# RaulAstudillo06/BOCF

Hardware: AMD Instinct MI355X
Metric: acquisition evals/sec (candidates x MC-samples/sec), uEI_noiseless batch call; GP-fit ms alongside (higher is better)
Workload: dtype f64; 1 GPU; BASELINE configs[2]: m=4 rbf-ARD GP, N=4096 d=8, S=1024 MC samples, C=65536 candidates, noise 1e-06, top-16 selection; N=4096, d=8, m=4, S=1024, C=65536, rccl_ranks_seen=0

## Files before the change

### bocf_amd/csrc/bocf_ctx.h

```cpp
#pragma once
#include "bocf_internal.h"
#include "chol_plan.h"
#include "predict_plan.h"
#include "../../include/bocf_hip.h"

#include <map>
#include <string>
#include <utility>
#include <vector>

void bocf_set_error(const char* text);
int bocf_launch_status();
int bocf_plan_cholesky(bocf_ctx* c, bool kinv, CholPlan* out);
int bocf_run_cholesky(bocf_ctx* c, const CholPlan& plan, bool counters_zeroed = false);
int bocf_run_trtri(bocf_ctx* c, bool early_done);
int bocf_comm_broadcast(bocf_ctx* c, double* buf, size_t count, int root);
int bocf_comm_group(bool start);
int bocf_comm_abort(bocf_ctx* c);
int bocf_comm_allreduce_sum(bocf_ctx* c, double* buf, size_t count);
#define fail bocf_fail
#define HIPCHK(expr)                                                         \
  do {                                                                       \
    hipError_t e_ = (expr);                                                  \
    if (e_ != hipSuccess) return fail(#expr, hipGetErrorString(e_));         \
// ... 8 lines not shown
static inline int nsplit_for(int Np, int Cpad, int m) {
  const int blocks = ((Cpad + 511) / 512) * m;
  int ns = 2048 / (blocks > 0 ? blocks : 1);
  if (ns < 1) ns = 1;
  const int maxs = Np / BOCF_TILE;
  if (ns > maxs) ns = maxs;
  return ns;
}



static_assert(PLAN_TILE == BOCF_TILE && PLAN_SMALL_N == BOCF_SMALL_N && PLAN_I8_SLICES == BOCF_I8_SLICES, "predict_plan.h mirrors bocf_internal.h");

struct DevBuf {
  void* p = nullptr;
  size_t cap = 0;
  int ensure(size_t bytes) {
    if (bytes <= cap) return 0;
    if (p) (void)hipFree(p);
    p = nullptr;
    cap = 0;
    hipError_t e = hipMalloc(&p, bytes);
    if (e != hipSuccess) return fail("hipMalloc", hipGetErrorString(e));
    cap = bytes;
    return 0;
  }
  void release() {
    if (p) (void)hipFree(p);
    p = nullptr;
    cap = 0;
  }
  template <typename T> T* as() const { return reinterpret_cast<T*>(p); }
};

struct bocf_ctx {
  int device = 0;
  hipStream_t stream = nullptr;
  void* pin_in = nullptr; void* pin_out = nullptr;
  size_t pin_in_cap = 0, pin_out_cap = 0;
  hipEvent_t ev_pin = nullptr;
  void* fit_pin = nullptr; size_t fit_pin_cap = 0;
  void* up_pin = nullptr; size_t up_pin_cap = 0, arena_used = 0;
  std::vector<hipEvent_t> ev_chol;
  hipStream_t s_res = nullptr, s_hi = nullptr, s_bulk = nullptr;
  DevBuf chol_flags;
  int chol_flags_used = 0;
  int chol_err_off = 0;
  CholOptions chol;
  int kinv_done = 0;
  int inverse_done = 0;
  int ncu = 0;
  int* tile_ctr = nullptr;
  unsigned long long* team_tl = nullptr;
  int res_cus = 0;
  int cu_masks_ok = 1;
  hipStream_t s_inv = nullptr;
  hipEvent_t ev_half = nullptr, ev_inv_early = nullptr;
  int early_inverse_started = 0;
  void* zeroed_R = nullptr; void* zeroed_RT = nullptr; int zeroed_Np = 0, zeroed_m = 0;
  int gated_off = 0;
  long long sched_timeouts = 0;
  int sched_retry = 0;
  long long fits_done = 0;
  int last_schedule = 0;
  int sched_m = 0;
  int force_sched_timeout = 0;
  int data_N = 0, data_d = 0, data_m = 0;
  int fused_infer = 1;
  int reuse_data = 0;
  int skip_mu_train = 0;
  DevBuf gpart, gout;
  DevBuf hmc_buf;
  double* infer_out = nullptr;
  size_t infer_out_cap = 0;
  bool fitted = false;
  bool canned = false;
  int N = 0, Np = 0, d = 0, m = 0, kernel_id = 0;
  long xs_stride = 0;
  std::vector<int> kernel_ids;
  std::vector<int> pending_ids;
  std::vector<KernHyp> hyp;
  std::vector<double> jitter;
  std::vector<int> last_info;
  DevBuf R32;
  bool r32_valid = false;
  int predict_f32 = 0;
  DevBuf Ri8, Ri8e, Ki8, Ki8e;
  bool ri8_valid = false;
  int predict_i8 = 0, i8_group = 0;
  DevBuf X, Xs, S, R, RT, E, ET, T, yc, tvec, rvec, dvec, alpha, lml, jit, hypd, info, mu_train;
  int C = 0;
  DevBuf Xc;
  long chunk = 65536;
  long workspace_mb = 24576;
  DevBuf Kstar, meanpart, sumsq, mean, var, acq, Vbuf, dmean, dvar, dacq, Vs, Ws;
  int pred_cap = 0;
  DevBuf theta, prob, best, params, Wt;
  std::vector<double> last_params;
  long long mu_epoch = 0;
  long long best_epoch = -1; int best_sig = -1;
  int S_mc = 0;
  bool have_acq = false;
  DevBuf prog_buf;
  UtilProg prog;
  DevBuf blk_idx, blk_val, out_idx, out_val;
  DevBuf eu_theta, eu_rows, eu_Z, eu_val, eu_grad;
// ... 120 lines not shown
```

### bocf_amd/csrc/bocf_internal.h

```cpp
#pragma once
#include <hip/hip_runtime.h>
#include <stdint.h>
#include "kern_dispatch.h"
#include "util_args.h"

#define BOCF_TILE 128
#define BOCF_MAX_FITS 1024

void bocf_note_launch(const char* kernel, hipError_t e);
#define BOCF_LAUNCH(kern, grid, block, shm, stream, ...)              \
  do {                                                                \
    hipLaunchKernelGGL(kern, grid, block, shm, stream, __VA_ARGS__);  \
    bocf_note_launch(#kern, hipGetLastError());                       \
  } while (0)
template <typename F>
static inline void bocf_launch_by_d(const char* kernel, int d, F f) {
  if (!bocf_dispatch_d(d, f)) bocf_note_launch(kernel, hipErrorInvalidValue);
}

__device__ __forceinline__ void dd_fma_acc(double& s, double& c, double a, double b) {
#pragma clang fp contract(off)
  const double p = a * b;
  const double e = __builtin_fma(a, b, -p);
  const double t = s + p;
// ... 1 lines not shown
  c += ((s - (t - z)) + (p - z)) + e;
  s = t;
}
__device__ __forceinline__ void dd_add_acc(double& s, double& c, double hi, double lo) {
#pragma clang fp contract(off)
  const double t = s + hi;
  const double z = t - s;
  c += ((s - (t - z)) + (hi - z)) + lo;
  s = t;
}

__device__ __forceinline__ double bocf_exp_nonpos_times(double x, double a) {
  x = __builtin_fmax(x, -1100.0);
  const double dn = __builtin_rint(x * 0x1.71547652b82fep+0);
  const double t = __builtin_fma(-dn, 0x1.abc9e3b39803fp-56, __builtin_fma(-dn, 0x1.62e42fefa39efp-1, x));
  double p = __builtin_fma(t, 0x1.ade156a5dcb37p-26, 0x1.28af3fca7ab0cp-22);
  p = __builtin_fma(t, p, 0x1.71dee623fde64p-19);
  p = __builtin_fma(t, p, 0x1.a01997c89e6b0p-16);
  p = __builtin_fma(t, p, 0x1.a01a014761f6ep-13);
  p = __builtin_fma(t, p, 0x1.6c16c1852b7b0p-10);
  p = __builtin_fma(t, p, 0x1.1111111122322p-7);
  p = __builtin_fma(t, p, 0x1.55555555502a1p-5);
  p = __builtin_fma(t, p, 0x1.5555555555511p-3);
  p = __builtin_fma(t, p, 0x1.000000000000bp-1);
  p = __builtin_fma(t, p, 1.0);
  p = __builtin_fma(t, p, 1.0);
  return __builtin_ldexp(a * p, (int)dn);
}
__device__ __forceinline__ double bocf_exp_nonpos(double x) { return bocf_exp_nonpos_times(x, 1.0); }

struct GemmArgs {
  const double* A;  long lda;  long strideA;
  const double* B;  long ldb;  long strideB;
  const double* Cin; double* Cout; long ldc; long strideC;
  int M, Ncols, K;
  int kb, krt, kct;
  int kbeg_rt, kbeg_ct;
  int batch1;
  long strideA2, strideB2, strideC2;
  int upper_only;
  int rt_desc;
  int ct_desc;
  int swizzle;
  int batch;
  int prefetch1;
  int stagger;
  int no_x3;
  int vprobe;
  double alpha, beta;
  double* sumsq;
  long strideSumsq;
  int* tile_ctr;
  int ncu;
};
void launch_gemm_f64(const GemmArgs& g, int batch, int epilogue, hipStream_t s);

struct GemmArgs32 {
  const float* A; long lda; long strideA;
  const float* B; long ldb; long strideB;
  int M, Ncols, K;
  double* sumsq; long strideSumsq;
  int tile128;
};
void launch_gemm_f32_sumsq(const GemmArgs32& g, int batch, hipStream_t s);
void launch_f64_to_f32(const double* src, float* dst, long n, hipStream_t s);

struct KernHyp {
  double variance;
  double noise;
  double ymean;
  double ls[BOCF_MAX_D];
  double jitter;
};

void launch_scale_inputs(const double* X, int n, int d, const KernHyp* hyp, int m, double* Xs, long strideXs, hipStream_t s);
void launch_build_train_kernel(const double* Xs, long strideXs, int N, int Np, int d, int kernel_id, const KernHyp* hyp,
                               const double* jitter, int add_diag, double* S, long strideS, int m, hipStream_t s, const int* kids = nullptr);
void launch_tile128(const double* A, long lda, long strideA, const double* B, long ldb, long strideB, double* C, long ldc, long strideC,
                    double alpha, double beta, int m, hipStream_t s, int ntiles = 1, int K = 128, int* done = nullptr);
#ifdef BOCF_PROBES
void dbg_tl_start();
void dbg_tl_dump(const char* path);
#endif
void set_potrf_scalar(int on);
void launch_potrf_diag(double* S, long strideS, int N, int Np, int p, double* E, double* ET, long strideE, int* info, int m, hipStream_t s,
                       int* done = nullptr);
void launch_gate(const int* f0, int n0, const int* f1, int n1, int* err, hipStream_t s);
void launch_signal(int* f, int add, hipStream_t s);
struct TeamArgs {
  double* S; double* RT; double* R; long strideS;
  double* E; double* ET; long strideE;
  int N, Np, nb;
  int* info;
  int* F; int fstride;
  int* err;
  int T;
  int p0, p1;
  int do_inverse;
  double* KI; int do_kinv;
  int crit_load;
  int stream;
  unsigned long long* tl;
};
void launch_chol_team(const TeamArgs& a, int m, hipStream_t s);
#define BOCF_INFER_MAX_D 16
void launch_infer128(const double* X, int N, int d, int kernel_id, const KernHyp* hyp, const double* yc, double* out, int m, hipStream_t s,
// ... 323 lines not shown
```

### bocf_amd/csrc/capi.hip

```cpp
#include "bocf_ctx.h"

#include <chrono>
#include <cmath>
#include <cstdio>
#include <cstdlib>
#include <cstring>
#include <string>
#include <vector>

static thread_local std::string g_err;
int bocf_fail(const char* what, const char* detail) {
  g_err = std::string(what) + ": " + (detail ? detail : "");
  return -1;
}
void bocf_set_error(const char* text) { g_err = text ? text : ""; }

static thread_local std::string g_launch_err;
void bocf_note_launch(const char* kernel, hipError_t e) {
  if (e != hipSuccess && g_launch_err.empty()) g_launch_err = std::string("launch of ") + kernel + ": " + hipGetErrorString(e);
}
int bocf_launch_status() {
  const hipError_t e = hipGetLastError();
  if (!g_launch_err.empty()) {
    g_err = g_launch_err;
// ... 38 lines not shown
  *out = c;
  return 0;
}

static void drop_events(bocf_ctx* c) {
  for (auto& pr : c->events) {
    (void)hipEventDestroy(pr.first);
    (void)hipEventDestroy(pr.second);
  }
  c->events.clear();
}

static void drop_phases(bocf_ctx* c) {
  for (auto& kv : c->phases)
    for (auto& pr : kv.second) {
      (void)hipEventDestroy(pr.first);
      (void)hipEventDestroy(pr.second);
    }
  c->phases.clear();
}

extern "C" void bocf_destroy(bocf_ctx* c) {
  if (!c) return;
  (void)hipSetDevice(c->device);
  (void)hipStreamSynchronize(c->stream);
  (void)bocf_comm_destroy(c);
  if (c->shard_helper) bocf_destroy(c->shard_helper);
  c->shard_helper = nullptr;
  if (c->ts_helper) bocf_destroy(c->ts_helper);
  c->ts_helper = nullptr;
  for (DevBuf& b : c->ts_F) b.release();
  for (DevBuf& b : c->pt_buf) b.release();
  drop_events(c);
  drop_phases(c);
  if (c->pin_in) (void)hipHostFree(c->pin_in);
  if (c->pin_out) (void)hipHostFree(c->pin_out);
  if (c->fit_pin) (void)hipHostFree(c->fit_pin);
  if (c->up_pin) (void)hipHostFree(c->up_pin);
  if (c->ev_pin) (void)hipEventDestroy(c->ev_pin);
  if (c->eu_pin) (void)hipHostFree(c->eu_pin);
  if (c->ev_eu_pin) (void)hipEventDestroy(c->ev_eu_pin);
  DevBuf* bufs[] = {&c->R32, &c->Ri8, &c->Ri8e, &c->Ki8, &c->Ki8e, &c->X, &c->Xs, &c->S, &c->R, &c->RT, &c->E, &c->ET, &c->T, &c->yc, &c->tvec, &c->alpha, &c->lml, &c->jit, &c->hypd,
                    &c->info, &c->mu_train, &c->rvec, &c->dvec, &c->hmc_buf, &c->Xc, &c->Kstar, &c->meanpart, &c->sumsq, &c->mean, &c->var, &c->acq, &c->Vbuf, &c->dmean, &c->dvar, &c->dacq, &c->Vs, &c->Ws, &c->theta,
                    &c->prob, &c->best, &c->params, &c->Wt, &c->blk_idx, &c->blk_val, &c->out_idx, &c->out_val, &c->gpart, &c->gout, &c->pack, &c->gidx,
                    &c->gval, &c->shard_meta, &c->chol_flags, &c->eu_theta, &c->eu_rows, &c->eu_Z, &c->eu_val, &c->eu_grad,
                    &c->ts_X, &c->ts_K, &c->ts_V, &c->ts_mp, &c->ts_mu, &c->ts_Z, &c->ts_jit, &c->ts_u, &c->ts_theta, &c->ts_params, &c->ts_out,
                    &c->kg_XA, &c->kg_VA, &c->kg_Wa, &c->kg_muA, &c->kg_s2A, &c->kg_nug, &c->kg_V, &c->kg_W, &c->kg_cov, &c->kg_s2c, &c->kg_dcov, &c->kg_dmean, &c->kg_dvar,
                    &c->kg_par, &c->kg_v0, &c->kg_astar, &c->kg_AB, &c->kg_out, &c->kg_dout, &c->prog_buf,
                    &c->pd_XP, &c->pd_VP, &c->pd_Wp, &c->pd_muP, &c->pd_cov, &c->pd_pack, &c->pd_QFG, &c->pd_par, &c->pd_best, &c->pd_T, &c->pd_muc, &c->pd_E,
                    &c->pt_E, &c->pt_g, &c->pt_rhs, &c->pt_tmp, &c->pt_nug, &c->pt_par, &c->pt_rows, &c->pt_tab, &c->pt_pv, &c->pt_pg, &c->pt_val, &c->pt_grad,
                    &c->cq_tab, &c->cq_par, &c->cq_best, &c->cq_nf, &c->cu_par, &c->cu_val, &c->cu_pof, &c->cu_grad, &c->cu_rng, &c->rf_dbl, &c->rf_int, &c->rf_x2, &c->rf_acq,
                    &c->loo_out, &c->loo_sum, &c->loo_shift, &c->loo_par, &c->loo_rows, &c->loo_val,
                    &c->jt_V, &c->jt_W, &c->jt_mu, &c->jt_cov, &c->jt_dmean, &c->jt_dvar, &c->jt_dcov, &c->jt_par, &c->jt_best, &c->jt_fl, &c->jt_E, &c->jt_dout,
                    &c->rk_par};
  for (DevBuf* b : bufs) b->release();
  if (c->infer_out) (void)hipHostFree(c->infer_out);
  if (c->tile_ctr) (void)hipFree(c->tile_ctr);
  for (hipEvent_t ev : c->ev_chol) (void)hipEventDestroy(ev);
  for (hipStream_t st : {c->s_res, c->s_hi, c->s_bulk, c->s_inv})
    if (st) (void)hipStreamDestroy(st);
  if (c->ev_half) (void)hipEventDestroy(c->ev_half);
  if (c->ev_inv_early) (void)hipEventDestroy(c->ev_inv_early);
  (void)hipStreamDestroy(c->stream);
  delete c;
}

struct OptDesc {
  const char* name;
  long long lo, hi;
  int kind;
  void (*set)(bocf_ctx*, long long);
  bool (*extra)(long long);
  const char* what;
};
static bool opt_lookahead_ok(long long v) { return v == -1 || v == 0 || v == 2; }
#ifdef BOCF_PROBES
static bool opt_swizzle_ok(long long v) { return v == -1 || v == 0 || v == 1 || (v >= 100 && v < 164) || (v >= 256 && v <= 258); }
static bool opt_potrf_ok(long long v) { return v == 0 || (v >= 11 && v <= 14); }
#else
static bool opt_swizzle_ok(long long v) { return v == -1 || v == 0 || v == 258; }
#endif
static const OptDesc g_options[] = {
    {"chunk", 128, 1 << 24, 0, [](bocf_ctx* c, long long v) { c->chunk = (long)round_up((int)v, 128); }, nullptr, "candidates per pass (rounded up to 128)"},
    {"workspace_mb", 1, 1 << 20, 0, [](bocf_ctx* c, long long v) { c->workspace_mb = (long)v; }, nullptr, "cap of the per-pass K* workspace"},
    {"profile", 0, 1, 0, [](bocf_ctx* c, long long v) { c->profile = v != 0; }, nullptr, "HIP events around the dominant kernel and the named phases"},
    {"predict_f32", 0, 1, 1, [](bocf_ctx* c, long long v) { c->predict_f32 = v != 0; }, nullptr, "fp32 variance contraction (BASELINE configs[4])"},
    {"i8_group", 0, 64, 0, [](bocf_ctx* c, long long v) { c->i8_group = (int)v; }, nullptr, "predict_i8: 0 = workgroups in blocks of 4 row-tile pairs x 8 column tiles per XCD; g >= 1 = bands of g pairs x all column tiles"},
    {"predict_i8", 0, 1, 1, [](bocf_ctx* c, long long v) { c->predict_i8 = v != 0; }, nullptr, "variance contraction in exact int8 products (six radix-254 digits per operand column, fp64 recombination)"},
    {"fused_infer", 0, 1, 0, [](bocf_ctx* c, long long v) { c->fused_infer = v != 0; }, nullptr, "one fused launch per inference for N <= 128"},
    {"reuse_data", 0, 1, 1, [](bocf_ctx* c, long long v) { c->reuse_data = v != 0; }, nullptr, "next fits reuse the resident X / Y"},
    {"skip_mu_train", 0, 1, 1, [](bocf_ctx* c, long long v) { c->skip_mu_train = v != 0; }, nullptr, "do not refresh the mean at the training inputs"},
    {"aggregate", 0, 8, 0, [](bocf_ctx* c, long long v) { c->chol.aggregate = (int)v; }, nullptr, "panels per trailing update (0 = by size)"},
    {"lookahead", -1, 2, 0, [](bocf_ctx* c, long long v) { c->chol.lookahead = (int)v; }, opt_lookahead_ok,
     "factorization schedule: -1 by size, 0 single stream, 2 reserved-CU chain"},
    {"team_fit", -1, 1, 0, [](bocf_ctx* c, long long v) { c->chol.team_fit = (int)v; }, nullptr, "factorization + inverse in one launch by resident workgroup teams (-1 = by size)"},
    {"team_panels", 1, 32, 0, [](bocf_ctx* c, long long v) { c->chol.team_panels = (int)v; }, nullptr, "team schedule above 8 panels: panels per team launch (one trailing update each)"},
    {"team_hybrid", 0, 2, 0, [](bocf_ctx* c, long long v) { c->chol.team_hybrid = (int)v; }, nullptr, "more than 24 panels: launched schedule for the first block rows, one team launch for the rest"},
    {"team_tail_share", 1, 8, 0, [](bocf_ctx* c, long long v) { c->chol.team_tail_share = (int)v; }, nullptr, "hybrid schedule: eighths of the compute units the tail's teams take"},
    {"team_whole_max", 2, 32, 0, [](bocf_ctx* c, long long v) { c->chol.team_whole_max = (int)v; }, nullptr, "panels up to which one team launch does the whole factorization and inverse"},
    {"team_stream", 0, 1, 0, [](bocf_ctx* c, long long v) { c->chol.team_stream = (int)v; }, nullptr, "teams: the critical tiles are formed underneath the diagonal blocks, 16 rows at a time"},
    {"team_crit_load", 0, 4096, 0, [](bocf_ctx* c, long long v) { c->chol.team_crit_load = (int)v; }, nullptr, "teams: critical-chain workgroups carry nothing else while the others get by with <= this many units each"},
    {"lookahead_min_nb", 2, 1 << 20, 0, [](bocf_ctx* c, long long v) { c->chol.lookahead_min_nb = (int)v; }, nullptr, "reserved-CU schedule from this many panels"},
    {"merge_x3", 0, 2, 0, [](bocf_ctx* c, long long v) { c->chol.merge_x3 = (int)v; }, nullptr, "second product of an inverse merge in the three-buffer kernel"},
    {"shard_fit", 0, 1, 0, [](bocf_ctx* c, long long v) { c->shard_fit = v != 0; }, nullptr, "output-sharded fit over the communicator"},
    {"trsm_wave", 0, 1, 0, [](bocf_ctx* c, long long v) { c->chol.trsm_wave = v != 0; }, nullptr, "row solves through the wave-level single-tile kernel"},
    {"overlap_inverse", -1, 1, 0, [](bocf_ctx* c, long long v) { c->chol.overlap_inverse = (int)v; }, nullptr, "early part of the inverse underneath the factorization (-1 = by size)"},
    {"small_path", 0, 1, 0, [](bocf_ctx* c, long long v) { c->small_path = v != 0; }, nullptr, "GEMV-shaped path for <= 16 candidates"},
// ... 156 lines not shown
                        s.Cpad, s.w, c->Kstar.as<double>(), s.Cpad, (long)c->Np * s.Cpad, mp, mp + p.mean_plane, nsplit_for(c->Np, s.Cpad, c->m), c->m,
                        p.kind == PRED_MEAN ? 0 : (p.kind == PRED_F32 ? 2 : 1), c->stream, BOCF_KIDS(c));
  if (!p.mean_with_var)
    launch_finalize_mean(mp, mp + p.mean_plane, p.nrt, s.Cpad, c->hypd.as<KernHyp>(), c->mean.as<double>(), p.ld, s.c0, s.Cn, c->m, c->stream);
}

static void predict_finalize(bocf_ctx* c, const PredictPass& s, int rows) {
  double* mp = c->meanpart.as<double>();
  launch_finalize_var(c->sumsq.as<double>(), rows, s.Cpad, c->hypd.as<KernHyp>(), s.flags, c->var.as<double>(), s.p.ld, s.c0, s.Cn, c->m, c->stream, mp,
                      mp + s.p.mean_plane, s.p.nrt, c->mean.as<double>());
}

static void contract_small(bocf_ctx* c, const PredictPass& s) {
  const int Np = c->Np, nc = small_width(s.Cn);
  const long strideS = (long)Np * Np;
  launch_gemv_small_t_mfma(c->R.as<double>(), strideS, Np, c->Kstar.as<double>(), s.Cpad, (long)Np * s.Cpad, c->Vs.as<double>(), c->sumsq.as<double>(),
                           s.Cpad, nc, c->m, c->stream);
  predict_finalize(c, s, Np / 16);
  if (!s.need_grad) return;
  launch_gemv_small_n_mfma(c->RT.as<double>(), strideS, Np, c->Vs.as<double>(), c->Ws.as<double>(), nc, c->m, c->stream);
  launch_grad_kernel(c->Xs.as<double>(), c->xs_stride, c->N, Np, c->d, c->kernel_id, c->hypd.as<KernHyp>(), c->Xc.as<double>(), s.c0, s.Cn, s.w,
                     c->Ws.as<double>(), nc, (long)Np * nc, c->dmean.as<double>(), c->dvar.as<double>(), s.p.ld, c->m, c->stream, BOCF_KIDS(c));
}

static void predict_gradients(bocf_ctx* c, const PredictPass& s) {
  const int Np = c->Np;
  GemmArgs v{};
  v.A = c->R.as<double>(); v.lda = Np; v.strideA = (long)Np * Np;
  v.B = c->Kstar.as<double>(); v.ldb = s.Cpad; v.strideB = (long)Np * s.Cpad;
  v.Cin = nullptr; v.Cout = c->Vbuf.as<double>(); v.ldc = s.Cpad; v.strideC = (long)Np * s.Cpad;
  v.M = Np; v.Ncols = s.Cpad; v.K = Np; v.kb = BOCF_TILE; v.krt = BOCF_TILE; v.rt_desc = 1; v.alpha = 1.0;
  launch_gemm_f64(v, c->m, 0, c->stream);
  GemmArgs w{};
  w.A = c->RT.as<double>(); w.lda = Np; w.strideA = (long)Np * Np;
  w.B = c->Vbuf.as<double>(); w.ldb = s.Cpad; w.strideB = (long)Np * s.Cpad;
  w.Cin = nullptr; w.Cout = c->Kstar.as<double>(); w.ldc = s.Cpad; w.strideC = (long)Np * s.Cpad;
  w.M = Np; w.Ncols = s.Cpad; w.K = Np; w.kb = Np; w.kbeg_rt = BOCF_TILE; w.alpha = 1.0;
  launch_gemm_f64(w, c->m, 0, c->stream);
  launch_grad_kernel(c->Xs.as<double>(), c->xs_stride, c->N, Np, c->d, c->kernel_id, c->hypd.as<KernHyp>(), c->Xc.as<double>(), s.c0, s.Cn, s.w,
                     c->Kstar.as<double>(), s.Cpad, (long)Np * s.Cpad, c->dmean.as<double>(), c->dvar.as<double>(), s.p.ld, c->m, c->stream, BOCF_KIDS(c));
}

static void contract_f64(bocf_ctx* c, const PredictPass& s) {
  const int Np = c->Np;
  GemmArgs g{};
  g.A = c->R.as<double>(); g.lda = Np; g.strideA = (long)Np * Np;
  g.B = c->Kstar.as<double>(); g.ldb = s.Cpad; g.strideB = (long)Np * s.Cpad;
  g.M = Np; g.Ncols = s.Cpad; g.K = Np; g.kb = BOCF_TILE; g.krt = BOCF_TILE; g.rt_desc = 1;
  g.swizzle = s.p.tiling(s.Cpad);
  g.vprobe = c->kstar_valu_probe;
  g.prefetch1 = c->prefetch1;
  g.sumsq = c->sumsq.as<double>(); g.strideSumsq = (long)s.p.nrt * s.Cpad;
  g.tile_ctr = c->tile_ctr; g.ncu = c->ncu;
  {
    KernelTimer t(c, s.Cn);
    launch_gemm_f64(g, c->m, 1, c->stream);
  }
  predict_finalize(c, s, s.p.nrt);
  if (s.need_grad) predict_gradients(c, s);
}

static void contract_f32(bocf_ctx* c, const PredictPass& s) {
  const int Np = c->Np;
  GemmArgs32 g{};
  g.A = c->R32.as<float>(); g.lda = Np; g.strideA = (long)Np * Np;
  g.B = c->Kstar.as<float>(); g.ldb = s.Cpad; g.strideB = (long)Np * s.Cpad;
  g.M = Np; g.Ncols = s.Cpad; g.K = Np;
  g.sumsq = c->sumsq.as<double>(); g.strideSumsq = (long)s.p.nrt * s.Cpad;
  g.tile128 = s.p.swizzle == 0;
  {
    KernelTimer t(c, s.Cn);
    launch_gemm_f32_sumsq(g, c->m, c->stream);
  }
  predict_finalize(c, s, s.p.nrt);
}

static void contract_i8(bocf_ctx* c, const PredictPass& s) {
  const int Np = c->Np;
  {
    KernelTimer t(c, s.Cn);
    launch_slice_operand(c->Kstar.as<double>(), s.Cpad, (long)Np * s.Cpad, Np, Np, s.Cpad, c->Ki8e.as<int>(), 0, c->Ki8.p, c->m, c->stream);
    launch_var_i8(c->Ri8.p, c->Ki8.p, Np, s.Cpad, c->Ri8e.as<int>(), c->Ki8e.as<int>(), c->sumsq.as<double>(), (long)s.p.nrt * s.Cpad, c->m, c->stream,
                  c->i8_group);
  }
  predict_finalize(c, s, s.p.nrt);
}

static int prepare_i8(bocf_ctx* c) {
  const int Np = c->Np, m = c->m;
  HIPCHK(hipMemsetAsync(c->Ri8e.p, 0x80, sizeof(int) * (size_t)m * Np, c->stream));
  launch_col_exponents(c->R.as<double>(), (long)Np * Np, Np, c->Ri8e.as<int>(), m, c->stream);
  launch_slice_operand(c->R.as<double>(), Np, (long)Np * Np, Np, Np, Np, c->Ri8e.as<int>(), Np, c->Ri8.p, m, c->stream);
  std::vector<int> eb(m);
  for (int j = 0; j < m; ++j) eb[j] = c->hyp[j].variance > 0.0 ? ilogb(c->hyp[j].variance) + 1 : 0;
  HIPCHK(hipMemcpyAsync(c->Ki8e.p, eb.data(), sizeof(int) * m, hipMemcpyHostToDevice, c->stream));
  HIPCHK(hipStreamSynchronize(c->stream));
  c->ri8_valid = true;
  return 0;
}

static int run_predict(bocf_ctx* c, int flags, bool need_var, bool need_grad = false, const double* w = nullptr) {
  const int C = c->C;
  if (C == 0) return 0;
  if (c->canned) {
    if (need_grad) return fail("predict", "a host-given posterior carries no gradients");
    return 0;
  }
  PredictPlanInput in;
  in.C = C; in.N = c->N; in.Np = c->Np; in.m = c->m; in.d = c->d; in.pred_cap = c->pred_cap;
  in.need_var = need_var; in.need_grad = need_grad;
// ... 495 lines not shown
```

### bocf_amd/csrc/gemm_f64.hip

```cpp
#include "bocf_internal.h"

typedef double v4d __attribute__((ext_vector_type(4)));
typedef double v2d __attribute__((ext_vector_type(2)));

#define BM 128
#define BM2 256
#define BN 128
#define BK 16
#define LDT 144
#define QCH 16

template <int EPI, int PF, int NW = 4>
__global__ __launch_bounds__(64 * NW, 2) void gemm_tn_f64_kernel(GemmArgs g) {
  constexpr int JB = NW == 4 ? 4 : 2;
  constexpr int SP = 16 / NW;
  __shared__ double lds[2][2][BK][LDT];

  const int nct = g.Ncols / BN;
  const int nrt = g.M / BM;
  int b = blockIdx.x;
  int rt, ct, batch;
#ifdef BOCF_PROBES
  if (g.swizzle >= 100) {
    const int RT = g.swizzle - 100;
// ... 314 lines not shown
    if (pos == 1 && kt + BK < kend) lstore(ra1, rb1, 1);
    if (on0) compute(0, 2, 4);
    if (pos == 2 && kt + BK < kend) lstore(ra1, rb1, 1);
    if (VPROBE != 2) __syncthreads();
    if (kt + BK >= kend) break;
    if (VPROBE != 4 && kt + 3 * BK < kend) gload(ra1, rb1, kt + 3 * BK);
    valu_probe(kt + BK);
    const bool on1 = kt + BK < my_kend;
    if (pos == 0 && kt + 2 * BK < kend) lstore(ra0, rb0, 0);
    if (on1) compute(1, 0, 2);
    if (pos == 1 && kt + 2 * BK < kend) lstore(ra0, rb0, 0);
    if (on1) compute(1, 2, 4);
    if (pos == 2 && kt + 2 * BK < kend) lstore(ra0, rb0, 0);
    if (VPROBE != 2) __syncthreads();
  }
  if (VPROBE && pacc == 1.2345e300) g.sumsq[0] = pacc;
  __syncthreads();
  double* red = &ldsA[0][0][0];
#pragma unroll
  for (int j = 0; j < 4; ++j) {
    double sq = 0.0;
#pragma unroll
    for (int i = 0; i < 4; ++i)
#pragma unroll
      for (int r = 0; r < 4; ++r) sq = __builtin_fma(acc[i][j][r], acc[i][j][r], sq);
    sq += __shfl_xor(sq, 16, 64);
    sq += __shfl_xor(sq, 32, 64);
    if (lq == 0) red[wr * 128 + wc * 64 + j * 16 + l15] = sq;
  }
  __syncthreads();
  if (tid < 256) {
    const int half = tid >> 7, col = tid & 127;
    double* out = g.sumsq + (long)batch * g.strideSumsq + (long)(rtA + half) * g.Ncols + (long)ct * BN;
    out[col] = red[(2 * half) * 128 + col] + red[(2 * half + 1) * 128 + col];
  }
}

#endif

template <int V>
struct IC {
  static constexpr int value = V;
};

#define LDA3 256
#define LDT3 128
template <int STORE, int QUEUE = 0>
__global__ __launch_bounds__(512, 1) void gemm_tn_f64_sumsq256x3_kernel(GemmArgs g) {
  static_assert(!(STORE && QUEUE), "the tile queue exists for the sum-of-squares epilogue only");
  __shared__ __attribute__((aligned(16))) double ldsA[3 * BK * LDA3];
  __shared__ __attribute__((aligned(16))) double ldsB[3 * BK * LDT3];
  __shared__ int next_tile;
  const int nct = g.Ncols / BN;
  const int nrt2 = g.M / BM2;
  int b = blockIdx.x;
  v2d ra0[4], rb0[2], ra1[4], rb1[2];
  bool primed = false;
  auto tile_of = [&](int t, int& rt2_, int& ct_, int& batch_) {
    const int per = nrt2 * nct;
    batch_ = t / per;
    const int rem = t - batch_ * per;
    rt2_ = rem / nct;
    ct_ = rem - rt2_ * nct;
  };
 for (;;) {
  int rt2, ct, batch;
  if (QUEUE) {
    tile_of(b, rt2, ct, batch);
  } else if (STORE) {
    const int per = nct * g.batch;
    rt2 = b / per;
    const int rem = b - rt2 * per;
    batch = rem / nct;
    ct = rem - batch * nct;
  } else {
    rt2 = b / nct;
    ct = b - rt2 * nct;
    batch = blockIdx.z;
  }
  if (g.rt_desc) rt2 = nrt2 - 1 - rt2;
  const int rtA = 2 * rt2;
  const int kend = BM2 * (rt2 + 1);
  const int k0 = kend - BM2;
  long offA = (long)batch * g.strideA, offB = (long)batch * g.strideB, offC = (long)batch * g.strideC;
  if (g.batch1 > 0) {
    const int z1 = batch % g.batch1, z2 = batch / g.batch1;
    offA = (long)z1 * g.strideA + (long)z2 * g.strideA2;
    offB = (long)z1 * g.strideB + (long)z2 * g.strideB2;
    offC = (long)z1 * g.strideC + (long)z2 * g.strideC2;
  }
  const double* A = g.A + offA + (long)rt2 * BM2;
  const double* B = g.B + offB + (long)ct * BN;
  const int tid = threadIdx.x;
  const int lane = tid & 63;
  const int wave = __builtin_amdgcn_readfirstlane(tid >> 6);
  const int wr = wave >> 1, wc = wave & 1;
  const int l15 = lane & 15, lq = lane >> 4;
  const int sl = tid & 15;
  const int arow = tid >> 7, swr = (tid >> 4) & 3, sh = (tid >> 6) & 1;
  const int brow = tid >> 6, sp = (tid >> 4) & 1, bw = (tid >> 5) & 1;
  const int stA = arow * LDA3 + sh * 128 + swr * 32 + sl * 2, stB = brow * LDT3 + bw * 64 + sp * 32 + sl * 2;
  const int fgA = lq * LDA3 + wr * 32 + l15 * 2, fgB = lq * LDT3 + wc * 64 + l15 * 2;
  int stA2h = (stA >> 1) + BK * LDA3, fgA2h = (fgA >> 1) + BK * LDA3;
  asm volatile("" : "+v"(stA2h), "+v"(fgA2h));
  const int stA2 = stA2h * 2, fgA2 = fgA2h * 2;

  v4d acc[4][4];
#pragma unroll
  for (int i = 0; i < 4; ++i)
#pragma unroll
    for (int j = 0; j < 4; ++j) acc[i][j] = (v4d){0.0, 0.0, 0.0, 0.0};
  const unsigned aoff = (unsigned)(((long)arow * g.lda + sh * 128 + swr * 16 + sl) * 8);
  const unsigned boff = (unsigned)(((long)brow * g.ldb + bw * 64 + sp * 32 + sl) * 8);
  const int lda8 = g.lda * 8, ldb8 = g.ldb * 8;
  auto fetch = [&](v2d (&ra)[4], v2d (&rb)[2], const double* pa, const double* pb) {
    const __amdgpu_buffer_rsrc_t resA = __builtin_amdgcn_make_buffer_rsrc(const_cast<double*>(pa), 0, -1, 0x00020000);
    const __amdgpu_buffer_rsrc_t resB = __builtin_amdgcn_make_buffer_rsrc(const_cast<double*>(pb), 0, -1, 0x00020000);
#pragma unroll
    for (int i = 0; i < 4; ++i) {
      ra[i][0] = __builtin_bit_cast(double, __builtin_amdgcn_raw_buffer_load_b64(resA, aoff, 4 * i * lda8, 0));
      ra[i][1] = __builtin_bit_cast(double, __builtin_amdgcn_raw_buffer_load_b64(resA, aoff + 512u, 4 * i * lda8, 0));
    }
#pragma unroll
    for (int i = 0; i < 2; ++i) {
      rb[i][0] = __builtin_bit_cast(double, __builtin_amdgcn_raw_buffer_load_b64(resB, boff, 8 * i * ldb8, 0));
      rb[i][1] = __builtin_bit_cast(double, __builtin_amdgcn_raw_buffer_load_b64(resB, boff + 128u, 8 * i * ldb8, 0));
    }
  };
  auto frag = [&](double (&a)[4], double (&bb)[4], auto bufc, auto ksc) {
    constexpr int BUF = decltype(bufc)::value, ROW = BUF * BK + decltype(ksc)::value * 4;
    const double* pa = BUF == 2 ? &ldsA[(ROW - 2 * BK) * LDA3 + fgA2] : &ldsA[ROW * LDA3 + fgA];
    const v2d a01 = *reinterpret_cast<const v2d*>(pa), a23 = *reinterpret_cast<const v2d*>(pa + 128);
    const v2d b01 = *reinterpret_cast<const v2d*>(&ldsB[ROW * LDT3 + fgB]), b23 = *reinterpret_cast<const v2d*>(&ldsB[ROW * LDT3 + fgB + 32]);
    a[0] = a01[0], a[1] = a01[1], a[2] = a23[0], a[3] = a23[1];
    bb[0] = b01[0], bb[1] = b01[1], bb[2] = b23[0], bb[3] = b23[1];
  };
  double xa[4], xb[4], ya[4], yb[4];
  auto interleave = [&](auto nmc) {
    constexpr int NM = decltype(nmc)::value;
#pragma unroll
    for (int ks = 0; ks < 4; ++ks) {
      const int nmem = ks < 3 ? 10 : 4;
      const int per = NM >= nmem ? 1 : (nmem + NM - 1) / NM;
      int done = 0;
// ... 58 lines not shown
    __syncthreads();
  };
  auto dstep = [&](v2d (&ra)[4], v2d (&rb)[2], int kt, int cur) {
    const int tau = (kt - k0) / BK;
    const int qmin = (tau - wr + 3) >> 2;
    const int nx = cur == 2 ? 0 : cur + 1, nn = nx == 2 ? 0 : nx + 1;
    const __amdgpu_buffer_rsrc_t resA = __builtin_amdgcn_make_buffer_rsrc(const_cast<double*>(pA), 0, -1, 0x00020000);
    const __amdgpu_buffer_rsrc_t resB = __builtin_amdgcn_make_buffer_rsrc(const_cast<double*>(pB), 0, -1, 0x00020000);
    const bool adv = kt + 5 * BK < kend;
    pA += adv ? tileA : 0;
    pB += adv ? tileB : 0;
    const double* fa_c = &ldsA[cur * (BK * LDA3) + fgA];
    const double* fb_c = &ldsB[cur * (BK * LDT3) + fgB];
    const double* fa_n = &ldsA[nx * (BK * LDA3) + fgA];
    const double* fb_n = &ldsB[nx * (BK * LDT3) + fgB];
    double* sa = &ldsA[nn * (BK * LDA3) + stA];
    double* sb = &ldsB[nn * (BK * LDT3) + stB];
    auto fragp = [&](double (&a)[4], double (&bb)[4], const double* pa, const double* pb, int ks) {
      const v2d a01 = *reinterpret_cast<const v2d*>(pa + ks * 4 * LDA3), a23 = *reinterpret_cast<const v2d*>(pa + ks * 4 * LDA3 + 128);
      const v2d b01 = *reinterpret_cast<const v2d*>(pb + ks * 4 * LDT3), b23 = *reinterpret_cast<const v2d*>(pb + ks * 4 * LDT3 + 32);
      a[0] = a01[0], a[1] = a01[1], a[2] = a23[0], a[3] = a23[1];
      bb[0] = b01[0], bb[1] = b01[1], bb[2] = b23[0], bb[3] = b23[1];
    };
    auto stld = [&](int i) {
      if (i < 4) {
        *reinterpret_cast<v2d*>(sa + 4 * i * LDA3) = ra[i];
        ra[i][0] = __builtin_bit_cast(double, __builtin_amdgcn_raw_buffer_load_b64(resA, aoff, 4 * i * lda8, 0));
        ra[i][1] = __builtin_bit_cast(double, __builtin_amdgcn_raw_buffer_load_b64(resA, aoff + 512u, 4 * i * lda8, 0));
      } else {
        *reinterpret_cast<v2d*>(sb + 8 * (i - 4) * LDT3) = rb[i - 4];
        rb[i - 4][0] = __builtin_bit_cast(double, __builtin_amdgcn_raw_buffer_load_b64(resB, boff, 8 * (i - 4) * ldb8, 0));
        rb[i - 4][1] = __builtin_bit_cast(double, __builtin_amdgcn_raw_buffer_load_b64(resB, boff + 128u, 8 * (i - 4) * ldb8, 0));
      }
    };
    auto k4 = [&](const double (&a)[4], const double (&bb)[4], int ks) {
#pragma unroll
      for (int q = 0; q < 4; ++q) {
        if (q >= qmin) {
#pragma unroll
          for (int j = 0; j < 4; ++j) acc[q][j] = __builtin_amdgcn_mfma_f64_16x16x4f64(a[q], bb[j], acc[q][j], 0, 0, 0);
        }
        if (ks < 3 && q < 2) stld(2 * ks + q);
      }
    };
    fragp(ya, yb, fa_c, fb_c, 1);
    k4(xa, xb, 0);
    fragp(xa, xb, fa_c, fb_c, 2);
    k4(ya, yb, 1);
    fragp(ya, yb, fa_c, fb_c, 3);
    k4(xa, xb, 2);
    fragp(xa, xb, fa_n, fb_n, 0);
    k4(ya, yb, 3);
    __syncthreads();
  };
  if (!(QUEUE && primed)) {
    fetch(ra0, rb0, A, B);
    fetch(ra1, rb1, A + tileA, B + tileB);
  }
#pragma unroll
  for (int i = 0; i < 4; ++i) *reinterpret_cast<v2d*>(&ldsA[4 * i * LDA3 + stA]) = ra0[i];
#pragma unroll
  for (int i = 0; i < 2; ++i) *reinterpret_cast<v2d*>(&ldsB[8 * i * LDT3 + stB]) = rb0[i];
  fetch(ra0, rb0, A + 2 * tileA, B + 2 * tileB);
#pragma unroll
  for (int i = 0; i < 4; ++i) *reinterpret_cast<v2d*>(&ldsA[(BK + 4 * i) * LDA3 + stA]) = ra1[i];
#pragma unroll
  for (int i = 0; i < 2; ++i) *reinterpret_cast<v2d*>(&ldsB[(BK + 8 * i) * LDT3 + stB]) = rb1[i];
  fetch(ra1, rb1, A + 3 * tileA, B + 3 * tileB);
  __syncthreads();
  frag(xa, xb, IC<0>(), IC<0>());
  const int nfull = k0 / BK, rounds = nfull / 6, rest = nfull - 6 * rounds;
  int kt = 0;
  for (int it = 0; it < rounds; ++it, kt += 6 * BK) {
    step(ra0, rb0, kt, IC<0>());
    step(ra1, rb1, kt + BK, IC<1>());
    step(ra0, rb0, kt + 2 * BK, IC<2>());
    step(ra1, rb1, kt + 3 * BK, IC<0>());
    step(ra0, rb0, kt + 4 * BK, IC<1>());
    step(ra1, rb1, kt + 5 * BK, IC<2>());
  }
  if (rest >= 2) {
    step(ra0, rb0, kt, IC<0>());
    step(ra1, rb1, kt + BK, IC<1>());
  }
  if (rest >= 4) {
    step(ra0, rb0, kt + 2 * BK, IC<2>());
    step(ra1, rb1, kt + 3 * BK, IC<0>());
  }
  int claimed = 0;
  if (QUEUE && tid == 0) claimed = (int)gridDim.x + atomicAdd(g.tile_ctr, 1);
  {
    int cur = rest == 0 ? 0 : (rest == 2 ? 2 : 1);
    for (kt = k0; kt < kend; kt += 2 * BK) {
      dstep(ra0, rb0, kt, cur);
      cur = cur == 2 ? 0 : cur + 1;
      dstep(ra1, rb1, kt + BK, cur);
      cur = cur == 2 ? 0 : cur + 1;
    }
  }
  if (STORE) {
    double* stage = ldsA;
    double* Cout = g.Cout + offC + (long)rt2 * BM2 * g.ldc + (long)ct * BN;
    const double alpha = g.alpha;
    __syncthreads();
#pragma unroll
    for (int pass = 0; pass < 4; ++pass) {
#pragma unroll
      for (int j = 0; j < 4; ++j)
#pragma unroll
        for (int r = 0; r < 4; ++r) stage[(16 * wr + 4 * r + lq) * LDT3 + wc * 64 + 16 * j + l15] = acc[pass][j][r];
      __syncthreads();
#pragma unroll
      for (int e = 0; e < 8; ++e) {
        const int rr = wave + 8 * e;
        v2d v = *reinterpret_cast<const v2d*>(&stage[rr * LDT3 + lane * 2]);
        v[0] *= alpha;
        v[1] *= alpha;
        *reinterpret_cast<v2d*>(Cout + (long)(64 * pass + rr) * g.ldc + lane * 2) = v;
      }
      __syncthreads();
    }
    return;
  }
  double* xfer = ldsA;
  double* red = ldsA + 4 * 4 * 2 * 64;
  int nb = 0;
  if (QUEUE && tid == 0) next_tile = claimed;
#pragma unroll 1
  for (int stage = 0; stage < 4; ++stage) {
    if (wr == stage) {
#pragma unroll
      for (int q = 0; q < 4; ++q)
#pragma unroll
        for (int j = 0; j < 4; ++j) {
          double* slot = xfer + ((q * 4 + j) * 2 + wc) * 64 + lane;
          double sq = stage == 0 ? 0.0 : *slot;
#pragma unroll
          for (int r = 0; r < 4; ++r) sq = __builtin_fma(acc[q][j][r], acc[q][j][r], sq);
          if (stage < 3) {
            *slot = sq;
          } else {
            sq += __shfl_xor(sq, 16, 64);
            sq += __shfl_xor(sq, 32, 64);
            if (lq == 0) red[q * 128 + wc * 64 + j * 16 + l15] = sq;
          }
        }
    }
    __syncthreads();
    if (QUEUE && stage == 0) {
      nb = __builtin_amdgcn_readfirstlane(next_tile);
      primed = nb < nrt2 * nct * g.batch;
      if (primed) {
        int nrt, nc, nz;
        tile_of(nb, nrt, nc, nz);
        if (g.rt_desc) nrt = nrt2 - 1 - nrt;
        const double* An = g.A + (long)nz * g.strideA + (long)nrt * BM2;
        const double* Bn = g.B + (long)nz * g.strideB + (long)nc * BN;
        fetch(ra0, rb0, An, Bn);
        fetch(ra1, rb1, An + tileA, Bn + tileB);
      }
    }
  }
  if (tid < 256) {
    const int half = tid >> 7, col = tid & 127;
    double* out = g.sumsq + (long)batch * g.strideSumsq + (long)(rtA + half) * g.Ncols + (long)ct * BN;
    out[col] = red[(2 * half) * 128 + col] + red[(2 * half + 1) * 128 + col];
  }
  if (!QUEUE) return;
  if (!primed) break;
  b = nb;
  __syncthreads();
 }
  if (threadIdx.x == 0 && atomicAdd(g.tile_ctr + 1, 1) == (int)gridDim.x - 1) {
    __hip_atomic_store(g.tile_ctr, 0, __ATOMIC_RELAXED, __HIP_MEMORY_SCOPE_AGENT);
    __hip_atomic_store(g.tile_ctr + 1, 0, __ATOMIC_RELAXED, __HIP_MEMORY_SCOPE_AGENT);
  }
}

void launch_gemm_f64(const GemmArgs& g0, int batch, int epilogue, hipStream_t s) {
  GemmArgs g = g0;
  g.batch = batch;
  const int nrt = g.M / BM, nct = g.Ncols / BN;
  if (nrt == 0 || nct == 0 || batch == 0) return;
  if (g.swizzle >= 256) {
    if (epilogue == 1 && !g.prefetch1 && g.M % BM2 == 0 && g.kbeg_rt == 0 && g.kbeg_ct == 0 && g.batch1 == 0) {
      const dim3 grid256((unsigned)((g.M / BM2) * nct), 1, (unsigned)batch);
#ifdef BOCF_PROBES
#define L256(V, A, B) BOCF_LAUNCH((gemm_tn_f64_sumsq256_kernel<V, A, B>), grid256, dim3(512), 0, s, g)
      if (g.swizzle != 258 || g.vprobe) {
        g.stagger = g.swizzle == 257 ? 1 : 0;
        if (g.vprobe == 1) L256(1, 2, 2);
        else if (g.vprobe == 2) L256(2, 2, 2);
        else if (g.vprobe == 3) L256(3, 2, 2);
        else if (g.vprobe == 4) L256(4, 2, 2);
        else if (g.stagger == 1) L256(0, 2, 0);
        else L256(0, 2, 2);
        return;
      }
#undef L256
#endif
      if (g.kb == BM && g.krt == BM && g.kct == 0 && g.K >= g.M) {
        const long tiles = (long)(g.M / BM2) * nct * batch;
        if (g.tile_ctr && g.ncu > 0 && tiles <= 0x7fffffffL - g.ncu)
          BOCF_LAUNCH((gemm_tn_f64_sumsq256x3_kernel<0, 1>), dim3((unsigned)(tiles < g.ncu ? tiles : g.ncu)), dim3(512), 0, s, g);
        else
          BOCF_LAUNCH((gemm_tn_f64_sumsq256x3_kernel<0>), grid256, dim3(512), 0, s, g);
        return;
      }
    }
    g.swizzle = 0;
  }
  if (epilogue == 0 && !g.no_x3 && !g.Cin && g.M % BM2 == 0 && g.M >= 2 * BM2 && g.kb == BM && g.krt == BM && g.kct == 0 && g.kbeg_rt == 0 && g.kbeg_ct == 0 &&
      g.K >= g.M && !g.upper_only && g.rt_desc && !g.ct_desc) {
    const dim3 grid256((unsigned)((g.M / BM2) * nct * batch), 1, 1);
    BOCF_LAUNCH((gemm_tn_f64_sumsq256x3_kernel<1>), grid256, dim3(512), 0, s, g);
    return;
  }
  if (epilogue == 3) {
    BOCF_LAUNCH((gemm_tn_f64_kernel<3, 1, 8>), dim3((unsigned)(nct * (nct + 1) / 2 * batch)), dim3(512), 0, s, g);
    return;
  }
  dim3 grid((unsigned)(nrt * nct), 1, (unsigned)batch);
#ifdef BOCF_PROBES
  if (g.swizzle >= 100 && (nct % 8 != 0 || nrt % (g.swizzle - 100) != 0)) g.swizzle = 0;
  if (g.swizzle >= 100) {
    grid = dim3((unsigned)(nrt * nct * batch), 1, 1);
  } else if (g.swizzle == 1) {
    const long ns = (long)((nrt + 7) / 8) * ((nct + 7) / 8) * batch;
    grid = dim3((unsigned)(((ns + 7) / 8) * 8 * 64), 1, 1);
  }
#else
  if (g.swizzle != 2) g.swizzle = 0;
#endif
  if (g.swizzle == 2) grid = dim3((unsigned)(nrt * nct * batch), 1, 1);
  if (epilogue == 0)
    BOCF_LAUNCH((gemm_tn_f64_kernel<0, 1, 8>), grid, dim3(512), 0, s, g);
  else if (g.prefetch1)
    BOCF_LAUNCH((gemm_tn_f64_kernel<1, 1>), grid, dim3(256), 0, s, g);
  else
    BOCF_LAUNCH((gemm_tn_f64_kernel<1, 2>), grid, dim3(256), 0, s, g);
}
```

Baseline: 1.088 billion evals/s.

## Extend 256-row sumsq GEMM to odd tile counts and restructure epilogue hand-over

Lets the fast 256-row variance sumsq kernel handle M not divisible by 256. It peels the leading 128-row tile into a separate small-kernel launch and offsets the rest by r0. The epilogue stage loop becomes a compile-time-unrolled lambda that batches LDS loads, FMAs and shuffles in groups to raise ILP. Probe-only cycle stamping, gated by BOCF_PROBES, is also added. For N=4096 the row count divides evenly, so only the epilogue restructuring affects this workload, at some risk of extra register pressure.

Measured after the change: 1.093 billion evals/s, median of 6. No clear change (+0.4%).

```diff
diff --git a/bocf_amd/csrc/bocf_ctx.h b/bocf_amd/csrc/bocf_ctx.h
--- a/bocf_amd/csrc/bocf_ctx.h
+++ b/bocf_amd/csrc/bocf_ctx.h
@@ -84,6 +84,7 @@
   int ncu = 0;
   int* tile_ctr = nullptr;
   unsigned long long* team_tl = nullptr;
+  DevBuf var_cycles;
   int res_cus = 0;
   int cu_masks_ok = 1;
   hipStream_t s_inv = nullptr;
diff --git a/bocf_amd/csrc/bocf_internal.h b/bocf_amd/csrc/bocf_internal.h
--- a/bocf_amd/csrc/bocf_internal.h
+++ b/bocf_amd/csrc/bocf_internal.h
@@ -77,6 +77,9 @@
   long strideSumsq;
   int* tile_ctr;
   int ncu;
+  int r0;
+  unsigned long long* cycles;
+  int cyc_tile;
 };
 void launch_gemm_f64(const GemmArgs& g, int batch, int epilogue, hipStream_t s);
 
diff --git a/bocf_amd/csrc/capi.hip b/bocf_amd/csrc/capi.hip
--- a/bocf_amd/csrc/capi.hip
+++ b/bocf_amd/csrc/capi.hip
@@ -114,7 +114,7 @@
                     &c->cq_tab, &c->cq_par, &c->cq_best, &c->cq_nf, &c->cu_par, &c->cu_val, &c->cu_pof, &c->cu_grad, &c->cu_rng, &c->rf_dbl, &c->rf_int, &c->rf_x2, &c->rf_acq,
                     &c->loo_out, &c->loo_sum, &c->loo_shift, &c->loo_par, &c->loo_rows, &c->loo_val,
                     &c->jt_V, &c->jt_W, &c->jt_mu, &c->jt_cov, &c->jt_dmean, &c->jt_dvar, &c->jt_dcov, &c->jt_par, &c->jt_best, &c->jt_fl, &c->jt_E, &c->jt_dout,
-                    &c->rk_par};
+                    &c->rk_par, &c->var_cycles};
   for (DevBuf* b : bufs) b->release();
   if (c->infer_out) (void)hipHostFree(c->infer_out);
   if (c->tile_ctr) (void)hipFree(c->tile_ctr);
@@ -377,10 +377,29 @@
   g.prefetch1 = c->prefetch1;
   g.sumsq = c->sumsq.as<double>(); g.strideSumsq = (long)s.p.nrt * s.Cpad;
   g.tile_ctr = c->tile_ctr; g.ncu = c->ncu;
+#ifdef BOCF_PROBES
+  const char* cyc_path = getenv("BOCF_VARIANCE_CYCLES");
+  if (cyc_path && !c->var_cycles.ensure(32 * sizeof(unsigned long long)) &&
+      hipMemsetAsync(c->var_cycles.p, 0, 32 * sizeof(unsigned long long), c->stream) == hipSuccess) {
+    const char* which = getenv("BOCF_VARIANCE_CYCLES_TILE");
+    g.cycles = c->var_cycles.as<unsigned long long>();
+    g.cyc_tile = which ? atoi(which) : 1;
+  }
+#endif
   {
     KernelTimer t(c, s.Cn);
     launch_gemm_f64(g, c->m, 1, c->stream);
   }
+#ifdef BOCF_PROBES
+  if (g.cycles) {
+    unsigned long long h[32] = {};
+    if (hipMemcpyAsync(h, g.cycles, sizeof(h), hipMemcpyDeviceToHost, c->stream) == hipSuccess && hipStreamSynchronize(c->stream) == hipSuccess)
+      if (FILE* f = fopen(cyc_path, "w")) {
+        for (int i = 0; i < 32; ++i) fprintf(f, "%d %llu\n", i, h[i]);
+        fclose(f);
+      }
+  }
+#endif
   predict_finalize(c, s, s.p.nrt);
   if (s.need_grad) predict_gradients(c, s);
 }
diff --git a/bocf_amd/csrc/gemm_f64.hip b/bocf_amd/csrc/gemm_f64.hip
--- a/bocf_amd/csrc/gemm_f64.hip
+++ b/bocf_amd/csrc/gemm_f64.hip
@@ -390,7 +390,8 @@
   __shared__ __attribute__((aligned(16))) double ldsB[3 * BK * LDT3];
   __shared__ int next_tile;
   const int nct = g.Ncols / BN;
-  const int nrt2 = g.M / BM2;
+  const int r0 = STORE ? 0 : g.r0;
+  const int nrt2 = (g.M - r0) / BM2;
   int b = blockIdx.x;
   v2d ra0[4], rb0[2], ra1[4], rb1[2];
   bool primed = false;
@@ -401,7 +402,29 @@
     rt2_ = rem / nct;
     ct_ = rem - rt2_ * nct;
   };
+#ifdef BOCF_PROBES
+  int tile_no = 0;
+#endif
  for (;;) {
+#ifdef BOCF_PROBES
+  const bool acct_wg = g.cycles && blockIdx.x == 0 && __builtin_amdgcn_readfirstlane((int)threadIdx.x >> 6) == 0;
+  const bool acct = acct_wg && tile_no == g.cyc_tile;
+  auto put = [&](int i, unsigned long long t) {
+    if ((threadIdx.x & 63) == 0) g.cycles[i] = t;
+  };
+  auto stamp = [&](int i) {
+    if (acct) put(i, __builtin_amdgcn_s_memtime());
+  };
+  if (acct_wg && tile_no == g.cyc_tile + 1) {
+    put(25, __builtin_amdgcn_s_memtime());
+    put(26, __builtin_amdgcn_s_memrealtime());
+  }
+  if (acct) put(1, __builtin_amdgcn_s_memrealtime());
+  stamp(0);
+  ++tile_no;
+#else
+  auto stamp = [](int) {};
+#endif
   int rt2, ct, batch;
   if (QUEUE) {
     tile_of(b, rt2, ct, batch);
@@ -417,8 +440,8 @@
     batch = blockIdx.z;
   }
   if (g.rt_desc) rt2 = nrt2 - 1 - rt2;
-  const int rtA = 2 * rt2;
-  const int kend = BM2 * (rt2 + 1);
+  const int rtA = r0 / BM + 2 * rt2;
+  const int kend = r0 + BM2 * (rt2 + 1);
   const int k0 = kend - BM2;
   long offA = (long)batch * g.strideA, offB = (long)batch * g.strideB, offC = (long)batch * g.strideC;
   if (g.batch1 > 0) {
@@ -427,7 +450,7 @@
     offB = (long)z1 * g.strideB + (long)z2 * g.strideB2;
     offC = (long)z1 * g.strideC + (long)z2 * g.strideC2;
   }
-  const double* A = g.A + offA + (long)rt2 * BM2;
+  const double* A = g.A + offA + r0 + (long)rt2 * BM2;
   const double* B = g.B + offB + (long)ct * BN;
   const int tid = threadIdx.x;
   const int lane = tid & 63;
@@ -592,6 +615,7 @@
     fragp(xa, xb, fa_n, fb_n, 0);
     k4(ya, yb, 3);
     __syncthreads();
+    stamp(4 + tau);
   };
   if (!(QUEUE && primed)) {
     fetch(ra0, rb0, A, B);
@@ -609,6 +633,7 @@
   fetch(ra1, rb1, A + 3 * tileA, B + 3 * tileB);
   __syncthreads();
   frag(xa, xb, IC<0>(), IC<0>());
+  stamp(2);
   const int nfull = k0 / BK, rounds = nfull / 6, rest = nfull - 6 * rounds;
   int kt = 0;
   for (int it = 0; it < rounds; ++it, kt += 6 * BK) {
@@ -627,6 +652,7 @@
     step(ra0, rb0, kt + 2 * BK, IC<2>());
     step(ra1, rb1, kt + 3 * BK, IC<0>());
   }
+  stamp(3);
   int claimed = 0;
   if (QUEUE && tid == 0) claimed = (int)gridDim.x + atomicAdd(g.tile_ctr, 1);
   {
@@ -666,46 +692,80 @@
   double* red = ldsA + 4 * 4 * 2 * 64;
   int nb = 0;
   if (QUEUE && tid == 0) next_tile = claimed;
-#pragma unroll 1
-  for (int stage = 0; stage < 4; ++stage) {
-    if (wr == stage) {
-#pragma unroll
-      for (int q = 0; q < 4; ++q)
-#pragma unroll
-        for (int j = 0; j < 4; ++j) {
-          double* slot = xfer + ((q * 4 + j) * 2 + wc) * 64 + lane;
-          double sq = stage == 0 ? 0.0 : *slot;
-#pragma unroll
-          for (int r = 0; r < 4; ++r) sq = __builtin_fma(acc[q][j][r], acc[q][j][r], sq);
-          if (stage < 3) {
-            *slot = sq;
-          } else {
-            sq += __shfl_xor(sq, 16, 64);
-            sq += __shfl_xor(sq, 32, 64);
-            if (lq == 0) red[q * 128 + wc * 64 + j * 16 + l15] = sq;
+  auto hand_over = [&](auto stagec) {
+    constexpr int ST = decltype(stagec)::value;
+    if (wr == ST) {
+      int xb = wc * 64 + lane, rb_ = wc * 64 + l15;
+      asm volatile("" : "+v"(xb), "+v"(rb_));
+#pragma unroll
+      for (int h = 0; h < 4; h += 2) {
+        double sq[2][4], t[2][4];
+#pragma unroll
+        for (int q = 0; q < 2; ++q)
+#pragma unroll
+          for (int j = 0; j < 4; ++j) sq[q][j] = ST == 0 ? 0.0 : xfer[((h + q) * 4 + j) * 128 + xb];
+#pragma unroll
+        for (int q = 0; q < 2; ++q)
+#pragma unroll
+          for (int j = 0; j < 4; ++j)
+#pragma unroll
+            for (int r = 0; r < 4; ++r) sq[q][j] = __builtin_fma(acc[h + q][j][r], acc[h + q][j][r], sq[q][j]);
+        if (ST < 3) {
+#pragma unroll
+          for (int q = 0; q < 2; ++q)
+#pragma unroll
+            for (int j = 0; j < 4; ++j) xfer[((h + q) * 4 + j) * 128 + xb] = sq[q][j];
+        } else {
+#pragma unroll
+          for (int q = 0; q < 2; ++q)
+#pragma unroll
+            for (int j = 0; j < 4; ++j) t[q][j] = __shfl_xor(sq[q][j], 16, 64);
+#pragma unroll
+          for (int q = 0; q < 2; ++q)
+#pragma unroll
+            for (int j = 0; j < 4; ++j) sq[q][j] += t[q][j];
+#pragma unroll
+          for (int q = 0; q < 2; ++q)
+#pragma unroll
+            for (int j = 0; j < 4; ++j) t[q][j] = __shfl_xor(sq[q][j], 32, 64);
+          if (lq == 0) {
+#pragma unroll
+            for (int q = 0; q < 2; ++q)
+#pragma unroll
+              for (int j = 0; j < 4; ++j) red[(h + q) * 128 + j * 16 + rb_] = sq[q][j] + t[q][j];
           }
         }
+      }
     }
     __syncthreads();
-    if (QUEUE && stage == 0) {
+    stamp(20 + ST);
+    if (QUEUE && ST == 0) {
       nb = __builtin_amdgcn_readfirstlane(next_tile);
       primed = nb < nrt2 * nct * g.batch;
       if (primed) {
         int nrt, nc, nz;
         tile_of(nb, nrt, nc, nz);
         if (g.rt_desc) nrt = nrt2 - 1 - nrt;
-        const double* An = g.A + (long)nz * g.strideA + (long)nrt * BM2;
+        const double* An = g.A + (long)nz * g.strideA + r0 + (long)nrt * BM2;
         const double* Bn = g.B + (long)nz * g.strideB + (long)nc * BN;
         fetch(ra0, rb0, An, Bn);
         fetch(ra1, rb1, An + tileA, Bn + tileB);
       }
     }
-  }
+  };
+  hand_over(IC<0>());
+  hand_over(IC<1>());
+  hand_over(IC<2>());
+  hand_over(IC<3>());
   if (tid < 256) {
     const int half = tid >> 7, col = tid & 127;
     double* out = g.sumsq + (long)batch * g.strideSumsq + (long)(rtA + half) * g.Ncols + (long)ct * BN;
     out[col] = red[(2 * half) * 128 + col] + red[(2 * half + 1) * 128 + col];
   }
+  stamp(24);
+#ifdef BOCF_PROBES
+  if (acct) put(27, (unsigned long long)(k0 / BK)), put(28, (unsigned long long)rt2), put(29, (unsigned long long)ct);
+#endif
   if (!QUEUE) return;
   if (!primed) break;
   b = nb;
@@ -720,11 +780,18 @@
 void launch_gemm_f64(const GemmArgs& g0, int batch, int epilogue, hipStream_t s) {
   GemmArgs g = g0;
   g.batch = batch;
+  g.r0 = 0;
   const int nrt = g.M / BM, nct = g.Ncols / BN;
   if (nrt == 0 || nct == 0 || batch == 0) return;
   if (g.swizzle >= 256) {
-    if (epilogue == 1 && !g.prefetch1 && g.M % BM2 == 0 && g.kbeg_rt == 0 && g.kbeg_ct == 0 && g.batch1 == 0) {
-      const dim3 grid256((unsigned)((g.M / BM2) * nct), 1, (unsigned)batch);
+    const int r0 = g.M % BM2;
+#ifdef BOCF_PROBES
+    const bool x3 = g.swizzle == 258 && !g.vprobe;
+#else
+    const bool x3 = true;
+#endif
+    if (epilogue == 1 && !g.prefetch1 && (r0 == 0 || (x3 && g.M > BM)) && g.kbeg_rt == 0 && g.kbeg_ct == 0 && g.batch1 == 0) {
+      const dim3 grid256((unsigned)(((g.M - r0) / BM2) * nct), 1, (unsigned)batch);
 #ifdef BOCF_PROBES
 #define L256(V, A, B) BOCF_LAUNCH((gemm_tn_f64_sumsq256_kernel<V, A, B>), grid256, dim3(512), 0, s, g)
       if (g.swizzle != 258 || g.vprobe) {
@@ -740,7 +807,14 @@
 #undef L256
 #endif
       if (g.kb == BM && g.krt == BM && g.kct == 0 && g.K >= g.M) {
-        const long tiles = (long)(g.M / BM2) * nct * batch;
+        if (r0) {
+          GemmArgs top = g;
+          top.M = BM;
+          top.swizzle = 0;
+          BOCF_LAUNCH((gemm_tn_f64_kernel<1, 2>), dim3((unsigned)nct, 1, (unsigned)batch), dim3(256), 0, s, top);
+          g.r0 = r0;
+        }
+        const long tiles = (long)((g.M - r0) / BM2) * nct * batch;
         if (g.tile_ctr && g.ncu > 0 && tiles <= 0x7fffffffL - g.ncu)
           BOCF_LAUNCH((gemm_tn_f64_sumsq256x3_kernel<0, 1>), dim3((unsigned)(tiles < g.ncu ? tiles : g.ncu)), dim3(512), 0, s, g);
         else
```
